# swkrueger/Thrifty

Hardware: AMD Instinct MI355X
Metric: IQ blocks/sec (16384-sample, 1024-chip template) (higher is better)
Workload: dtype f32; 1 GPU; BASELINE configs[1]: block_len=16384 history=4096 1023-chip Gold template, dense, 1048576 blocks/GPU resident in HBM as u8 IQ; variant=default, blocks_per_launch_batch=32768, templates=1, thresholds=15*snr, parallelism=block-shard x1, handles_per_gpu=2, detections_gathered=1048576

## Files before the change

### include/thrifty_hip.h

```cpp
#ifndef THRIFTY_HIP_H
#define THRIFTY_HIP_H

#include <stddef.h>
#include <stdint.h>

#ifdef __cplusplus
extern "C" {
#endif

#define THR_ABI_VERSION 11

#define THR_OK 0
#define THR_ERR_ARG (-1)
#define THR_ERR_DEVICE (-2)
#define THR_ERR_STATE (-3)
#define THR_ERR_INDEX (-4)

#define THR_FLAG_CARRIER 1u
#define THR_FLAG_CORR 2u
#define THR_FLAG_INDEX_ERROR 4u

#define THR_FLAG_FIT_UNCONVERGED 16u
#define THR_FLAG_INT_OFFSET 8u

// ... 168 lines not shown
int thr_run_gate_card(thr_handle* h, const char* text, size_t text_len, const thr_gate_run_opts* opts,
                      thr_gate_run_stats* stats);

typedef struct thr_extract thr_extract;
int thr_extract_create(thr_handle* h, double max_offset, thr_extract** out);
void thr_extract_destroy(thr_extract* x);
int thr_extract_reset(thr_extract* x);
int thr_extract_feed(thr_extract* x, const void* samples, int format, const int64_t* block_idx,
                     const double* timestamps, size_t n_blocks, thr_record* out);
int thr_extract_feed_card(thr_extract* x, const char* text, size_t text_len, const int64_t* payload_off,
                          const int64_t* block_idx, const double* timestamps, size_t n_blocks, thr_record* out);
int thr_extract_feed_stream(thr_extract* x, const uint8_t* stream, size_t n_bytes, int64_t first_block_idx,
                            const double* timestamps, thr_record* out, size_t out_capacity, size_t* n_blocks_out);
int thr_extract_submit_card(thr_extract* x, const char* text, size_t text_len, const int64_t* payload_off,
                            const int64_t* block_idx, const double* timestamps, size_t n_blocks, thr_record* out,
                            uint64_t* ticket);
int thr_extract_submit_stream(thr_extract* x, const uint8_t* stream, size_t n_bytes, int64_t first_block_idx,
                              double timestamp, thr_record* out, size_t out_capacity, size_t* n_blocks_out,
                              uint64_t* ticket);
int thr_extract_result(thr_extract* x, thr_record* best, double* timestamp, double* template_out, size_t capacity,
                       uint64_t* n_qualifying);
int thr_run_extract_card(thr_handle* h, const char* text, size_t text_len, const thr_run_opts* opts,
                         thr_extract* x, thr_run_stats* stats);
int thr_run_extract_stream(thr_handle* h, const uint8_t* stream, size_t n_bytes, int64_t first_block_idx,
                           const thr_run_opts* opts, thr_extract* x, thr_run_stats* stats);

typedef struct thr_survey thr_survey;
int thr_survey_create(thr_handle* h, int integrate, thr_survey** out);
void thr_survey_destroy(thr_survey* s);
int thr_survey_reset(thr_survey* s);
int thr_survey_shift(const thr_survey* s, int* shift);
int thr_survey_pending(const thr_survey* s, uint64_t* blocks_fed, uint64_t* blocks_in_open_interval);
int thr_survey_feed(thr_survey* s, const uint8_t* samples, size_t n_blocks, uint64_t* sums, uint64_t* spec_sum,
                    uint64_t* hist, size_t cap_intervals, size_t* n_intervals);
int thr_survey_feed_stream(thr_survey* s, const uint8_t* stream, size_t n_bytes, uint64_t* sums, size_t sums_capacity,
                           size_t* n_blocks, uint64_t* spec_sum, uint64_t* hist, size_t cap_intervals,
                           size_t* n_intervals);
int thr_debug_survey_geometry(const thr_survey* s, int* tile_blocks, int* workgroups, int* fused);

typedef struct thr_chip_record {
    int32_t sample;
    uint32_t flags;
    float energy, noise;
    double offset;
} thr_chip_record;
int thr_chipscan(thr_handle* h, const void* samples, int format, size_t n_blocks,
                 const uint8_t* chips, int n_chips,
                 const int32_t* lengths, size_t n_lengths,
                 thr_chip_record* out, thr_record* carrier_out );
int thr_debug_chipscan_geometry(thr_handle* h, size_t n_lengths, int* candidates_per_chunk, int* paired);
int thr_debug_chipscan_budget(thr_handle* h, size_t bank_bytes);
int thr_debug_chipscan_times(thr_handle* h, double* ms_out );

int thr_get_settings(const thr_handle* h, thr_settings* out);

int thr_compact_device(thr_handle* h, const thr_record* d_in, size_t n_records,
                       thr_record* d_out, size_t* n_kept);

#define THR_N_KERNEL_SLOTS 5
int thr_profile_enable(thr_handle* h, int on);
int thr_profile_read(thr_handle* h, double ms[THR_N_KERNEL_SLOTS],
                     int64_t launches[THR_N_KERNEL_SLOTS]);
const char* thr_kernel_name(int slot);

int thr_debug_correlate_geom(thr_handle* h, int* rows_lo, int* rows_hi);
#define THR_WHY_SECTIONED 0
#define THR_WHY_PATH 1
#define THR_WHY_VARIANT 2
#define THR_WHY_STDDEV 3
#define THR_WHY_GEOMETRY 4
#define THR_WHY_BLOCK_LEN 5
typedef struct thr_path_info {
    int32_t n_sections, section_len;
    int32_t rows_lo, rows_hi;
    int32_t why_unsectioned;
    int32_t n_templates;
    char carrier_kernel[48];
    char correlate_kernel[48];
    char text[256];
} thr_path_info;
int thr_get_path_info(thr_handle* h, thr_path_info* out);

int thr_debug_sections(thr_handle* h, int* n_sections, int* section_len);
int thr_debug_window(thr_handle* h, size_t out[4]);
int thr_debug_window_times(thr_handle* h, double out[6]);
int thr_debug_pipe_times(thr_handle* h, double out[16]);
int thr_debug_live_resources(int64_t out[4]);
int thr_debug_fft(thr_handle* h, const void* samples, int format, size_t n_blocks,
                  float* spectra_out );
int thr_debug_stage(thr_handle* h, const void* samples, int format, size_t n_blocks,
                    int template_id, float* shifted_fft_out ,
                    float* corr_out );
int thr_debug_stage_offsets(thr_handle* h, const void* samples, int format, size_t n_blocks,
                            int template_id, const double* carrier_offset ,
                            float* shifted_fft_out, float* corr_out);

typedef struct thr_freq_range {
    int32_t rxid;
    int32_t txid;
    double lo;
    double hi;
} thr_freq_range;

int thr_identify(int device_id, size_t n, const int32_t* rxid, const int32_t* block,
                 const double* timestamp, const int32_t* carrier_bin, const double* carrier_offset,
                 const double* energy, const thr_freq_range* map, size_t n_map, int32_t* txid_out,
                 uint8_t* keep_out, int64_t* kept_order_out, size_t* n_kept_out);

int thr_match(int device_id, size_t n, const int32_t* rxid, const int32_t* txid,
              const double* timestamp, const double* energy, double window, int min_match,
              int64_t* match_ptr_out, int64_t* match_idx_out, size_t* n_matches_out,
              int64_t* miss_out, size_t* n_misses_out,
              int64_t* collision_out, size_t* n_collisions_out);
int thr_debug_match_times(double* ms_out );

int thr_tdoa(int device_id, size_t n_det, const int32_t* rx, const double* timestamp, const double* soa,
             const double* energy, const double* noise, size_t n_matches, const int64_t* match_ptr,
             const int64_t* match_idx, const int32_t* match_beacon, int n_rx, int n_beacons,
             const double* dist, double window, double sample_rate, int deg, size_t n_tasks,
             int32_t* row_rx_out, int64_t* row_det_out, double* row_val_out, size_t* n_rows_out,
             int64_t* group_id_out, int64_t* group_ptr_out, size_t* n_groups_out,
             int64_t* fail_out, size_t* n_fail_out, int32_t* n_window_out, int32_t* n_kept_out);
int thr_debug_tdoa_times(double* ms_out );

#define THR_POS_OK 0
#define THR_POS_UNDERDETERMINED 1
#define THR_POS_UNCONVERGED 2
#define THR_POS_AT_BOUND 3
#define THR_POS_NONFINITE 4
int thr_pos(int device_id, size_t n_groups, const int64_t* group_ptr, const int32_t* row_rx0,
            const int32_t* row_rx1, const double* row_tdoa, const double* row_snr, int n_rx, int dims,
            const double* rx_coords, const int32_t* first_two_rx, const double* x0, int max_iter,
            double* pos_out, double* dop_out, double* snr_out, int32_t* status_out, int32_t* iters_out);
int thr_debug_pos_times(double* ms_out );

typedef struct thr_post_settings {
    const thr_freq_range* map;
    size_t n_map;
    double match_window;
    int32_t min_match;
    int32_t n_rx;
    const int32_t* rx_ids;
    int32_t dims;
    int32_t n_beacons;
    const double* rx_coords;
    int32_t first_two_rx[2];
    const int32_t* beacon_ids;
    const double* dist;
    double tdoa_window;
    double sample_rate;
    int32_t deg;
    int32_t max_iter;
    double x0[2];
    int32_t tdoa_as_text;
    int32_t reserved;
} thr_post_settings;
typedef struct thr_post_counts {
    size_t kept, matches, match_entries, misses, collisions, tasks, rows, groups, failures;
} thr_post_counts;
typedef struct thr_post thr_post;
#define THR_POST_TXID 0
#define THR_POST_KEEP 1
#define THR_POST_KEPT_ORDER 2
#define THR_POST_MATCH_PTR 3
#define THR_POST_MATCH_IDX 4
#define THR_POST_MISSES 5
// ... 65 lines not shown
```

### thrifty_amd/_native.py

```python
from __future__ import annotations

import atexit
import ctypes as C
import os
import weakref

import numpy as np

HERE = os.path.dirname(os.path.abspath(__file__))
LIB_PATH = os.environ.get("THRIFTY_HIP_LIB") or os.path.join(HERE, "libthriftyhip.so")

THR_IN_U8 = 0
THR_IN_C64 = 1
FLAG_CARRIER = 1
FLAG_CORR = 2
FLAG_INDEX_ERROR = 4
FLAG_INT_OFFSET = 8
FLAG_FIT_UNCONVERGED = 16
N_KERNEL_SLOTS = 5

ABI_VERSION = 11

EXPORTS = [
    "thr_abi_version", "thr_last_error", "thr_create", "thr_destroy", "thr_detect",
    "thr_create_preshift", "thr_create_fastdet", "thr_create_ex", "thr_plan_sections", "thr_host_register", "thr_host_unregister", "thr_input_window", "thr_detect_card", "thr_detect_stream", "thr_detect_stream_device", "thr_detect_device", "thr_sync", "thr_set_stream", "thr_compact_device",
    "thr_profile_enable", "thr_profile_read", "thr_kernel_name", "thr_debug_fft",
    "thr_debug_stage", "thr_debug_stage_offsets", "thr_identify", "thr_frame_card",
    "thr_submit", "thr_submit_card", "thr_submit_stream", "thr_collect", "thr_inputs_consumed", "thr_poll",
    "thr_set_stream_default", "thr_format_toad",
    "thr_run_card", "thr_run_stream", "thr_get_settings", "thr_input_window_ex", "thr_input_window_release", "thr_detect_offsets", "thr_set_wait_mode", "thr_debug_window", "thr_debug_window_times", "thr_debug_correlate_geom", "thr_debug_sections", "thr_debug_pipe_times", "thr_get_path_info",
    "thr_gate", "thr_gate_stream", "thr_gate_card", "thr_gate_slot_stride", "thr_format_card",
    "thr_run_gate_stream", "thr_run_gate_card",
    "thr_extract_create", "thr_extract_destroy", "thr_extract_reset", "thr_extract_feed", "thr_extract_feed_card",
    "thr_extract_feed_stream", "thr_extract_submit_card", "thr_extract_submit_stream", "thr_extract_result",
    "thr_run_extract_card", "thr_run_extract_stream",
    "thr_match", "thr_debug_match_times",
    "thr_tdoa", "thr_debug_tdoa_times",
    "thr_pos", "thr_debug_pos_times",
    "thr_postdetect", "thr_post_fetch", "thr_post_free", "thr_debug_post_times",
    "thr_debug_live_resources",
    "thr_survey_create", "thr_survey_destroy", "thr_survey_reset", "thr_survey_shift", "thr_survey_pending",
    "thr_survey_feed", "thr_survey_feed_stream", "thr_debug_survey_geometry",
    "thr_chipscan", "thr_debug_chipscan_geometry", "thr_debug_chipscan_budget", "thr_debug_chipscan_times",
    "thr_toadstats", "thr_tstats_fetch", "thr_tstats_free", "thr_debug_toadstats_times", "thr_debug_toadstats_geometry",
]
ERR_ARG, ERR_DEVICE, ERR_STATE, ERR_INDEX = -1, -2, -3, -4
VARIANT_DEFAULT, VARIANT_PRESHIFT, VARIANT_FASTDET, VARIANT_GATE = 0, 1, 2, 3
INTERPOLATORS = {"parabolic": 0, "none": 1, "gaussian": 2, "cosine": 3}
PATHS = {"auto": 0, "multipass": 1, "unsectioned": 2, "generic_rows": 3, "unsectioned_generic_rows": 4}
MAX_IN_FLIGHT = 3
TOAD_LINE_MAX = 384
CARD_HEADER_MAX = 48


class ThrSettings(C.Structure):
    _fields_ = [
        ("block_len", C.c_int32), ("history_len", C.c_int32),
        ("n_templates", C.c_int32), ("template_len", C.c_int32),
        ("templates", C.POINTER(C.c_double)),
        ("carrier_len", C.c_int32), ("carrier_window", C.c_int32 * 2),
        ("carrier_thresh", C.c_double * 3), ("corr_thresh", C.c_double * 3),
        ("device_id", C.c_int32), ("max_batch", C.c_int32),
    ]


class ThrPathInfo(C.Structure):
    _fields_ = [
        ("n_sections", C.c_int32), ("section_len", C.c_int32), ("rows_lo", C.c_int32), ("rows_hi", C.c_int32),
        ("why_unsectioned", C.c_int32), ("n_templates", C.c_int32),
        ("carrier_kernel", C.c_char * 48), ("correlate_kernel", C.c_char * 48), ("text", C.c_char * 256),
    ]


WHY_UNSECTIONED = ("sectioned", "path", "variant", "stddev", "geometry", "block_len")


class ThrRunOpts(C.Structure):
    _fields_ = [
        ("struct_bytes", C.c_uint32), ("batch_blocks", C.c_int32), ("out_fd", C.c_int32),
        ("with_rxid", C.c_int32), ("rxid", C.c_int64), ("with_txid", C.c_int32),
        ("carrier_offset_mode", C.c_int32), ("timestamp", C.c_double),
        ("rec_out", C.c_void_p), ("rec_capacity", C.c_size_t),
    ]


class ThrRunStats(C.Structure):
    _fields_ = [
        ("blocks", C.c_uint64), ("detections", C.c_uint64), ("batches", C.c_uint64),
        ("bytes_in", C.c_uint64), ("text_bytes", C.c_uint64), ("index_error_at", C.c_uint64),
        ("index_error_block", C.c_int64), ("index_error_bin", C.c_int32), ("reserved_", C.c_int32),
        ("total_s", C.c_double), ("frame_s", C.c_double), ("submit_s", C.c_double), ("wait_s", C.c_double),
        ("format_s", C.c_double), ("write_s", C.c_double),
    ]

    def as_dict(self):
        return {name: getattr(self, name) for name, _ in self._fields_ if name != "reserved_"}


class ThrGateRunOpts(C.Structure):
    _fields_ = [
        ("struct_bytes", C.c_uint32), ("batch_blocks", C.c_int32), ("out_fd", C.c_int32), ("skip", C.c_int32),
        ("timestamp", C.c_double), ("rec_out", C.c_void_p), ("rec_capacity", C.c_size_t),
    ]


class ThrGateRunStats(C.Structure):
    _fields_ = [
        ("blocks", C.c_uint64), ("passed", C.c_uint64), ("batches", C.c_uint64), ("bytes_in", C.c_uint64),
        ("text_bytes", C.c_uint64), ("total_s", C.c_double), ("frame_s", C.c_double), ("gate_s", C.c_double),
        ("wait_s", C.c_double), ("format_s", C.c_double), ("write_s", C.c_double),
    ]

    def as_dict(self):
# ... 636 lines not shown
        if buf is None:
            _check(self._lib, self._lib.thr_input_window(self._h, None, 0))
            self._window = None
            return
        if getattr(self, "_window", None) is not None:
            _check(self._lib, self._lib.thr_input_window(self._h, None, 0))
            self._window = None
        arr = np.frombuffer(buf, dtype=np.uint8)
        _check(self._lib, self._lib.thr_input_window_ex(self._h, arr.ctypes.data, arr.size,
                                                        int(populate_threads), int(segment_bytes)))
        self._window = arr

    def input_window_release(self):
        self._lib.thr_input_window_release.argtypes = [C.c_void_p]
        _check(self._lib, self._lib.thr_input_window_release(self._h))

    def _run_opts(self, out_fd, rxid, with_txid, carrier_offset_mode, batch_blocks, rec_out, timestamp=None):
        o = ThrRunOpts()
        o.struct_bytes = C.sizeof(ThrRunOpts)
        o.batch_blocks = int(batch_blocks or 0)
        o.out_fd = -1 if out_fd is None else int(out_fd)
        o.with_rxid, o.rxid = (0, 0) if rxid is None else (1, int(rxid))
        o.with_txid = int(bool(with_txid))
        o.carrier_offset_mode = int(carrier_offset_mode)
        o.timestamp = float("nan") if timestamp is None else float(timestamp)
        if rec_out is not None:
            assert rec_out.dtype == RECORD_DTYPE and rec_out.flags.c_contiguous
            o.rec_out, o.rec_capacity = rec_out.ctypes.data, rec_out.size
        return o

    def _run_done(self, rc, stats):
        out = stats.as_dict()
        out["index_error"] = rc == ERR_INDEX
        if rc != 0 and rc != ERR_INDEX:
            raise NativeError("libthriftyhip: %s (code %d)" % (self._lib.thr_last_error().decode(), rc),
                              rc, out)
        return out

    def _run(self, data, call):
        buf = np.frombuffer(data, dtype=np.uint8)
        st = ThrRunStats()
        rc = call(buf.ctypes.data if buf.size else None, buf.size, C.byref(st))
        del buf
        return self._run_done(rc, st)

    def run_card(self, text, out_fd=None, rxid=None, with_txid=False, carrier_offset_mode=0,
                 batch_blocks=0, rec_out=None):
        o = self._run_opts(out_fd, rxid, with_txid, carrier_offset_mode, batch_blocks, rec_out)
        return self._run(text, lambda ptr, n, st: self._lib.thr_run_card(self._h, ptr, n, C.byref(o), st))

    def run_stream(self, stream, first_block_idx=0, out_fd=None, rxid=None, with_txid=False,
                   carrier_offset_mode=0, batch_blocks=0, rec_out=None, timestamp=None):
        o = self._run_opts(out_fd, rxid, with_txid, carrier_offset_mode, batch_blocks, rec_out, timestamp)
        return self._run(stream, lambda ptr, n, st: self._lib.thr_run_stream(self._h, ptr, n, int(first_block_idx),
                                                                             C.byref(o), st))

    def debug_window(self):
        out = (C.c_size_t * 4)()
        self._lib.thr_debug_window.argtypes = [C.c_void_p, C.c_size_t * 4]
        _check(self._lib, self._lib.thr_debug_window(self._h, out))
        return tuple(int(v) for v in out)

    def correlate_geom(self):
        lo, hi = C.c_int(-1), C.c_int(-1)
        self._lib.thr_debug_correlate_geom.argtypes = [C.c_void_p, C.POINTER(C.c_int), C.POINTER(C.c_int)]
        _check(self._lib, self._lib.thr_debug_correlate_geom(self._h, C.byref(lo), C.byref(hi)))
        return lo.value, hi.value

    def path_info(self):
        info = ThrPathInfo()
        self._lib.thr_get_path_info.argtypes = [C.c_void_p, C.POINTER(ThrPathInfo)]
        _check(self._lib, self._lib.thr_get_path_info(self._h, C.byref(info)))
        return {"n_sections": info.n_sections, "section_len": info.section_len,
                "rows": (info.rows_lo, info.rows_hi), "why_unsectioned": WHY_UNSECTIONED[info.why_unsectioned],
                "n_templates": info.n_templates, "carrier_kernel": info.carrier_kernel.decode(),
                "correlate_kernel": info.correlate_kernel.decode(), "text": info.text.decode()}

    def sections(self):
        n, ln = C.c_int(0), C.c_int(0)
        self._lib.thr_debug_sections.argtypes = [C.c_void_p, C.POINTER(C.c_int), C.POINTER(C.c_int)]
        _check(self._lib, self._lib.thr_debug_sections(self._h, C.byref(n), C.byref(ln)))
        return n.value, ln.value

    def debug_pipe_times(self):
        out = (C.c_double * 16)()
        self._lib.thr_debug_pipe_times.argtypes = [C.c_void_p, C.c_double * 16]
        _check(self._lib, self._lib.thr_debug_pipe_times(self._h, out))
        keys = ("grow_s", "h2d_s", "meta_s", "launch_s", "d2h_s", "chunks", "event_s", "fill_s")
        res = dict(zip(keys, (float(v) for v in out[:8])))
        res.update(("max_" + k, float(v)) for k, v in zip(keys, out[8:]) if k != "chunks")
        return res

    def debug_window_times(self):
        out = (C.c_double * 6)()
        self._lib.thr_debug_window_times.argtypes = [C.c_void_p, C.c_double * 6]
        _check(self._lib, self._lib.thr_debug_window_times(self._h, out))
        keys = ("populate_s", "register_s", "unregister_s", "acquire_wait_s", "acquire_waits", "pageable_copies")
        return dict(zip(keys, (float(v) for v in out)))

    def set_wait_mode(self, sleeping):
        self._lib.thr_set_wait_mode.argtypes = [C.c_void_p, C.c_int]
        _check(self._lib, self._lib.thr_set_wait_mode(self._h, int(bool(sleeping))))

    def collect(self, ticket):
        _check(self._lib, self._lib.thr_collect(self._h, ticket.id))
        ticket.keep = None
        return ticket.out

    def inputs_consumed(self, ticket):
        _check(self._lib, self._lib.thr_inputs_consumed(self._h, ticket.id))
        ticket.keep = None

    def poll(self, ticket):
        done = C.c_int(0)
        _check(self._lib, self._lib.thr_poll(self._h, ticket.id, C.byref(done)))
        return bool(done.value)

    def detect_stream_device(self, d_stream, n_blocks, d_out, d_block_idx=None):
        _check(self._lib, self._lib.thr_detect_stream_device(self._h, d_stream, d_block_idx,
                                                             n_blocks, d_out))

    def detect_device(self, d_samples, fmt, n_blocks, d_out, d_block_idx=None):
        _check(self._lib, self._lib.thr_detect_device(self._h, d_samples, fmt, d_block_idx,
                                                      n_blocks, d_out))

    def compact_device(self, d_in, n_records, d_out):
        kept = C.c_size_t(0)
        _check(self._lib, self._lib.thr_compact_device(self._h, d_in, n_records, d_out,
                                                       C.byref(kept)))
        return kept.value

    def sync(self):
        _check(self._lib, self._lib.thr_sync(self._h))

    def set_stream(self, stream_ptr):
        if not stream_ptr:
            _check(self._lib, self._lib.thr_set_stream_default(self._h))
        else:
            _check(self._lib, self._lib.thr_set_stream(self._h, stream_ptr))

    def use_own_stream(self):
        _check(self._lib, self._lib.thr_set_stream(self._h, None))

    def profile_enable(self, every=1):
        _check(self._lib, self._lib.thr_profile_enable(self._h, int(every)))

    def profile_read(self):
        ms = (C.c_double * N_KERNEL_SLOTS)()
        cnt = (C.c_int64 * N_KERNEL_SLOTS)()
        _check(self._lib, self._lib.thr_profile_read(self._h, ms, cnt))
        return {self._lib.thr_kernel_name(i).decode(): (ms[i], cnt[i])
                for i in range(N_KERNEL_SLOTS)}

    def debug_fft(self, blocks):
        a, fmt = self._as_input(blocks)
        out = np.zeros((a.shape[0], self.block_len), dtype=np.complex64)
        _check(self._lib, self._lib.thr_debug_fft(self._h, a.ctypes.data, fmt, a.shape[0],
                                                  out.ctypes.data))
        return out

    def debug_stage(self, blocks, template_id=0, carrier_offset=None):
        a, fmt = self._as_input(blocks)
        xhat = np.zeros((a.shape[0], self.block_len), dtype=np.complex64)
        corr = np.zeros((a.shape[0], self.block_len), dtype=np.complex64)
        off = None
        if carrier_offset is not None:
# ... 475 lines not shown
```

### thrifty_amd/csrc/detect16k_sec.hip

```cpp
#include <hip/hip_runtime.h>

#include <algorithm>

#include "detect_common.hpp"
#include "fft_regs.hpp"
#include "kernel_util.hpp"
#include "passes_w8.hpp"

namespace thr {

using namespace k16;

namespace {

constexpr int QN = 4096;
constexpr int QR = 4;
constexpr int QA = 8;
constexpr int QT = 128;
constexpr int QDATA = QR * ROW;
constexpr int Q_DYN = 128, Q_PH = 192, Q_NPH = 98;
constexpr size_t QLDS = size_t(QDATA) * sizeof(cpx) + 1024;
#ifndef THR_Q_MULTI_FORM
#define THR_Q_MULTI_FORM 1
#endif
constexpr int Q_MULTI_FORM = THR_Q_MULTI_FORM;

template <int FMT>
struct RawQ;

template <>
struct RawQ<THR_IN_U8> {
    unsigned q[QR * QA / 2];
    __device__ __forceinline__ void load(const void* __restrict__ sec, int t) {
        const unsigned char* p = static_cast<const unsigned char*>(sec) + unsigned(t) * (QA * 2);
#pragma unroll
        for (int n1 = 0; n1 < QR; ++n1)
            __builtin_memcpy(&q[n1 * (QA / 2)], p + n1 * 2048, QA * 2);
    }
    __device__ __forceinline__ void pair(int n1, int i, cpx& a, cpx& b) const {
        const unsigned w = q[n1 * (QA / 2) + i];
        constexpr float sc = 1.0f / 128.0f, of = -127.4f / 128.0f;
        a = __builtin_elementwise_fma(cpx{float(w & 0xffu), float((w >> 8) & 0xffu)}, cpx{sc, sc}, cpx{of, of});
        b = __builtin_elementwise_fma(cpx{float((w >> 16) & 0xffu), float(w >> 24)}, cpx{sc, sc}, cpx{of, of});
    }
};

template <>
struct RawQ<THR_IN_C64> {
    const f4* p;
    __device__ __forceinline__ void load(const void* __restrict__ sec, int t) {
        p = reinterpret_cast<const f4*>(sec) + size_t(t) * (QA / 2);
    }
    __device__ __forceinline__ void pair(int n1, int i, cpx& a, cpx& b) const {
        const f4 w = p[n1 * 512 + i];
        a = cpx{w.x, w.y};
        b = cpx{w.z, w.w};
    }
};

template <class RAW>
__device__ __forceinline__ void q_pass1(cpx* lds, const RAW& raw, int t, const float2* __restrict__ rpow,
                                        const cpx (&qk)[QR], const cpx* u) {
    const int m0 = t * QA;
    cpx* out = lds + (m0 >> 5) * CHUNK + (m0 & 31);
    static_for<QA / 2>([&](auto I) {
        constexpr int i = decltype(I)::value;
        cpx v0[QR], v1[QR];
#pragma unroll
        for (int n1 = 0; n1 < QR; ++n1) {
            raw.pair(n1, i, v0[n1], v1[n1]);
            if (n1 != 0) {
                const cpx r = cpx{rpow[n1].x, rpow[n1].y};
                v0[n1] = cmul_uniform(v0[n1], r);
                v1[n1] = cmul_uniform(v1[n1], r);
            }
        }
        dft_reg<QR, -1>(v0);
        dft_reg<QR, -1>(v1);
        static_for<QR>([&](auto K) {
            constexpr int k1 = decltype(K)::value;
            const f4 uu = *reinterpret_cast<const f4*>(u + k1 * QA + 2 * i);
            cpx w0, w1, y0, y1;
            cmul2(qk[k1], cpx{uu.x, uu.y}, qk[k1], cpx{uu.z, uu.w}, w0, w1);
            cmul2(v0[brev(k1, QR)], w0, v1[brev(k1, QR)], w1, y0, y1);
            *reinterpret_cast<f4*>(out + k1 * ROW + 2 * i) = f4{y0.x, y0.y, y1.x, y1.y};
        });
    });
}

__device__ __forceinline__ void q_pass2(cpx* lds, const cpx (&cw)[R2]) {
    const int t = opaque_tid();
    cpx* base = lds + (t >> 5) * ROW + (t & 31);
    cpx v[R2];
#pragma unroll
    for (int n2 = 0; n2 < R2; ++n2) v[n2] = lds_b64(base + n2 * CHUNK);
    dft_reg<R2, -1>(v);
    static_for<R2 / 2>([&](auto K) {
        constexpr int k2 = 2 * decltype(K)::value;
        cpx y0 = v[brev(k2, R2)], y1 = v[brev(k2 + 1, R2)];
        if constexpr (k2 != 0)
            cmul2(y0, cw[k2], y1, cw[k2 + 1], y0, y1);
        else
            y1 = cmul(y1, cw[1]);
        base[k2 * CHUNK] = y0;
        base[(k2 + 1) * CHUNK] = y1;
    });
}

__device__ __forceinline__ void q_passA(cpx* lds, cpx* z, const cpx (&cw)[R2]) {
    const int t = opaque_tid();
    cpx v[R3];
    static_for<R3>([&](auto K) {
        constexpr int k3 = decltype(K)::value;
        v[k3] = z[brev(k3, R3)];
    });
    dft_reg<R3, +1>(v);
    f4* dst = reinterpret_cast<f4*>(lds + (t >> 5) * ROW + (t & 31) * CHUNK);
    static_for<R3 / 2>([&](auto J) {
        constexpr int j = decltype(J)::value;
        cpx y0 = v[brev(2 * j, R3)], y1 = v[brev(2 * j + 1, R3)];
        if constexpr (j != 0)
            cmulc2(y0, cw[2 * j], y1, cw[2 * j + 1], y0, y1);
        else
            y1 = cmulc(y1, cw[1]);
        dst[j] = f4{y0.x, y0.y, y1.x, y1.y};
    });
}

template <int H>
__device__ __forceinline__ void q_cw_half(const f4* __restrict__ ctp, f4 (&w)[R2 / 4]) {
    const char* p = reinterpret_cast<const char*>(ctp);
    const unsigned off = unsigned(opaque_tid() & 31) * 16u;
    static_for<R2 / 4>([&](auto J) {
        constexpr int j = decltype(J)::value;
        w[j] = *reinterpret_cast<const f4*>(p + (off + unsigned((H * (R2 / 4) + j) * 512)));
    });
}

__device__ __forceinline__ void q_pass2_ld(cpx* lds, const f4* __restrict__ ctp) {
// ... 148 lines not shown
        });
    });
}

struct QPhasor {
    cpx wq;
    float ang;
    cpx seg;
};
__device__ __forceinline__ QPhasor q_phasor_fetch(const ShiftParams* __restrict__ sp, int seg,
                                                  const cpx* __restrict__ twn, int t) {
    QPhasor r;
    const int tt = t < Q_NPH ? t : 0;
    const int u = tt - 66;
    const int m = tt < 64 ? 8 * tt : tt < 66 ? 512 * (tt - 64) : (u & 7);
    const int si = sp->si_mod - (tt < 66 ? 0 : 4 * (u >> 3));
    r.wq = twn[(si * m) & (N - 1)];
    r.ang = 6.283185307179586f * (sp->sf_over_n * float(m));
    r.seg = cpx{sp->segc0[seg].x, sp->segc0[seg].y};
    return r;
}
__device__ __forceinline__ void q_phasor_store(const QPhasor& r, int t, cpx* sc_ph) {
    if (t < Q_NPH) {
        float sn, cs;
        sincos_small(r.ang, &sn, &cs);
        cpx v = cmul(cconj(r.wq), cpx{cs, sn});
        if (t >= 64 && t < 66) v = cmul(v, r.seg);
        sc_ph[t] = v;
    }
}

template <int FMT, bool GENERIC_ROWS, int MULTI>
__global__ __launch_bounds__(QT) __attribute__((amdgpu_waves_per_eu(2))) void k_correlate_4k(
    const void* __restrict__ samples, DevCfg cfg, const cpx* __restrict__ ctab,
    const cpx* __restrict__ twn, const f4* __restrict__ tspec, const ShiftParams* __restrict__ shifts,
    const int* __restrict__ work_list, const int* __restrict__ work_count,
    CorrStats* __restrict__ seg_stats, const f4* __restrict__ ctp, f4* __restrict__ park) {
    extern __shared__ __attribute__((aligned(16))) unsigned char smem_raw[];
    cpx* lds = reinterpret_cast<cpx*>(smem_raw);
    unsigned char* sc_red = reinterpret_cast<unsigned char*>(lds + QDATA);
    cpx* sc_ph = reinterpret_cast<cpx*>(sc_red + Q_PH);
    int* sc_dyn = reinterpret_cast<int*>(sc_red + Q_DYN);

    const size_t blk_bytes = cfg.blk_stride;
    const int n_seg = cfg.n_seg;
    const int n_work = *work_count * n_seg;
    constexpr int kSampleBytes = FMT == THR_IN_U8 ? 2 : 8;
    const cpx* gtw = static_cast<const cpx*>(cfg.gtw);
    int parity = 0;

    cpx cw[R2];
    if constexpr (MULTI != 1) {
        const int c = opaque_tid() & 31;
        cw[0] = cpx{1.f, 0.f};
#pragma unroll
        for (int k = 1; k < R2; ++k) cw[k] = ctab[k * 32 + c];
    }
    f4* const slot = MULTI == 2 ? park + size_t(blockIdx.x) * (QN / 2) + opaque_tid() : nullptr;
    const int n_tpl = MULTI ? cfg.n_templates : 1;

    cpx bk[QR];
    {
        const int m0 = opaque_tid() * QA;
        bk[0] = cpx{1.f, 0.f};
#pragma unroll
        for (int k1 = 1; k1 < QR; ++k1) bk[k1] = gtw[k1 * (16 / QR) * 1024 + m0];
    }

    auto item_entry = [&](int wi) -> int { return n_seg == 4 ? wi >> 2 : wi / n_seg; };
    auto item_at = [&](int wi) -> int {
        const int e = item_entry(wi);
        return (work_list[e] << 3) | (wi - e * n_seg);
    };
    auto item_samples = [&](int item) -> const unsigned char* {
        return static_cast<const unsigned char*>(samples) + size_t(item >> 3) * blk_bytes +
               size_t(cfg.seg_start[item & 7]) * kSampleBytes;
    };

    const int G = int(gridDim.x);
    const int tk = n_work <= 2 * G ? 1 : n_seg;
    auto last_of_ticket = [&](int wi) -> bool {
        return tk == 1 ? true : tk == 4 ? ((wi + 1) & 3) == 0 : (wi + 1) % tk == 0;
    };
    bool static_ticket = true;
    int wi0 = int(blockIdx.x) * tk, wi_nxt;
    if (!last_of_ticket(wi0)) {
        wi_nxt = wi0 + 1;
    } else {
        wi_nxt = (int(blockIdx.x) + G) * tk;
        static_ticket = false;
    }
    RawQ<FMT> cur;
    int it_next = wi0 < n_work ? item_at(wi0) : 0;
    int it_next2 = wi_nxt < n_work ? item_at(wi_nxt) : 0;
    int blk_next2 = it_next2 >> 3, seg_next2 = it_next2 & 7;
    if (wi0 < n_work) {
        cur.load(item_samples(it_next), opaque_tid());
        q_phasor_store(q_phasor_fetch(shifts + (it_next >> 3), it_next & 7, twn, opaque_tid()), opaque_tid(), sc_ph);
    }
    __syncthreads();
    int* dyn_ctr = const_cast<int*>(work_count) + 1;
    f4 tq[R3 / 2];
    auto request_tq = [&](int tpl) {
        const char* ts = reinterpret_cast<const char*>(tspec + size_t(tpl) * (QN / 2));
        const unsigned off = unsigned(opaque_tid()) * 16u;
        static_for<R3 / 2>([&](auto J) {
            constexpr int j = decltype(J)::value;
            tq[j] = *reinterpret_cast<const f4*>(ts + (off + unsigned(j * (QT * 16))));
        });
    };
    if constexpr (MULTI != 0) request_tq(0);
    for (int wi = wi0, iter = 0; wi < n_work; ++iter) {
#ifdef THR_DEV
        const bool tl_on = blockIdx.x == 0 && iter == 40 && cfg.timeline != nullptr;
#endif
        THR_STAMP(0);
        const int item = it_next;
        const int b = item >> 3, seg = item & 7;
        const int t = opaque_tid();
        const ShiftParams* sp = shifts + b;
        const bool need_ticket = last_of_ticket(wi_nxt);
        int wi_dyn = 0;
#ifdef THR_Q_STATIC
        (void)dyn_ctr;
        wi_dyn = (wi_nxt + 1) / tk - 1 - G;
#else
        if (t == 0 && need_ticket && !static_ticket) wi_dyn = atomicAdd(dyn_ctr, 1);
#endif
        RawQ<FMT> nxt = cur;
        const bool more = wi_nxt < n_work;
        if (more) {
            it_next = (blk_next2 << 3) | seg_next2;
            nxt.load(item_samples(it_next), t);
        }
        const QPhasor ph = q_phasor_fetch(shifts + (it_next >> 3), it_next & 7, twn, t);
        THR_STAMP(1);
        {
            cpx qk[QR];
            qk[0] = cmul(sc_ph[64 + (t >> 6)], sc_ph[t & 63]);
#pragma unroll
            for (int k1 = 1; k1 < QR; ++k1) qk[k1] = cmul(qk[0], bk[k1]);
            q_pass1(lds, cur, t, sp->rpow, qk, sc_ph + 66);
        }
        cur = nxt;
        THR_STAMP(2);
        if (t == 0)
            *sc_dyn = !need_ticket ? wi_nxt + 1
                                   : (static_ticket ? int(blockIdx.x) + G : 2 * G + wi_dyn) * tk;
        if (need_ticket) static_ticket = false;
        THR_STAMP(3);
        __syncthreads();
        THR_STAMP(4);
        const int wi_nxt2 = __builtin_amdgcn_readfirstlane(*sc_dyn);
        if (wi_nxt2 < n_work) {
            const int e = item_entry(wi_nxt2);
            blk_next2 = work_list[e];
            seg_next2 = wi_nxt2 - e * n_seg;
        }
        wi = wi_nxt;
        wi_nxt = wi_nxt2;
        if (more) q_phasor_store(ph, t, sc_ph);
        if constexpr (MULTI == 0) request_tq(0);
        if constexpr (MULTI == 1)
            q_pass2_ld(lds, ctp);
        else
            q_pass2(lds, cw);
        __builtin_amdgcn_sched_barrier(0);
        THR_STAMP(5);
        cpx z[R3];
        cpx xh[R3];
        fwd_pass3(lds, xh);
        THR_STAMP(6);
        if constexpr (MULTI == 2) {
            static_for<R3 / 2>([&](auto J) {
                constexpr int j = decltype(J)::value;
                slot[j * QT] = f4{xh[brev(2 * j, R3)].x, xh[brev(2 * j, R3)].y, xh[brev(2 * j + 1, R3)].x,
                                  xh[brev(2 * j + 1, R3)].y};
            });
        }
        static_for<R3 / 2>([&](auto J) {
            constexpr int j = decltype(J)::value;
            const f4 q = tq[j];
            cmul2(xh[brev(2 * j, R3)], cpx{q.x, q.y}, xh[brev(2 * j + 1, R3)], cpx{q.z, q.w},
                  z[brev(2 * j, R3)], z[brev(2 * j + 1, R3)]);
        });
      for (int tpl = 0;;) {
        if constexpr (MULTI == 1)
            q_passA_ld(lds, z, ctp);
        else
            q_passA(lds, z, cw);
        __builtin_amdgcn_sched_barrier(0);
        THR_STAMP(7);
        if constexpr (THR_Q_PAIRED_B)
            q_passB<MULTI == 1>(lds, reinterpret_cast<const f4*>(gtw + 16 * 1024));
        else if constexpr (MULTI == 1)
            q_passB_ld(lds, gtw, (opaque_tid() >> 5) * (16 / QR));
        else
            inv_passB<true>(lds, gtw, (opaque_tid() >> 5) * (16 / QR));
        THR_STAMP(8);
        __syncthreads();
        THR_STAMP(9);
        cpx c[QR * QA];
        q_passC(lds, opaque_tid(), c);
        THR_STAMP(10);

        const int w_lo = cfg.seg_lo[seg], w_hi = cfg.seg_hi[seg];
        const int m0 = t * QA;
        float pw[QR * QA];
        float wmax;
        unsigned lag;
        const bool whole_rows = !GENERIC_ROWS && w_lo <= 1 && w_hi >= 3 * 1024 && w_hi <= 3 * 1024 + 1;
        if (whole_rows) {
            float tmax = -1.0f;
            static_for<3 * QA / 2 + 1>([&](auto Q) {
                constexpr int q = 2 * decltype(Q)::value;
                pw[q] = cnorm(c[q]);
                pw[q + 1] = cnorm(c[q + 1]);
            });
            const float e0 = m0 >= w_lo ? pw[0] : -1.f;
            const float e24 = (m0 == 0 && w_hi > 3 * 1024) ? pw[24] : -1.f;
            tmax = __builtin_fmaxf(e0, e24);
            static_for<3 * QA / 2>([&](auto Q) {
                constexpr int q = 2 * decltype(Q)::value;
                if constexpr (q == 0)
                    tmax = __builtin_fmaxf(tmax, pw[1]);
                else
                    tmax = __builtin_fmaxf(tmax, __builtin_fmaxf(pw[q], pw[q + 1]));
            });
#pragma unroll
            for (int q = 3 * QA + 2; q < QR * QA; ++q) pw[q] = 0.f;
            wmax = wave_max_f32(tmax);
            int first = 63;
            first = e24 == wmax ? 24 : first;
            static_for<3 * QA - 1>([&](auto Q) {
                constexpr int q = 3 * QA - 1 - decltype(Q)::value;
                first = pw[q] == wmax ? q : first;
            });
            first = e0 == wmax ? 0 : first;
            lag = first == 63 ? 0xFFFFFFFFu : unsigned((first >> 3) * 1024 + m0 + (first & 7));
        } else {
            const unsigned win_w = unsigned(w_hi - w_lo);
            float ew[QR * QA];
            float tmax = -1.0f;
            static_for<QR * QA / 2>([&](auto Q) {
                constexpr int q = 2 * decltype(Q)::value;
                constexpr int n1 = q / QA, j = q % QA;
                pw[q] = cnorm(c[q]);
                pw[q + 1] = cnorm(c[q + 1]);
                const int n = n1 * 1024 + m0 + j;
                ew[q] = unsigned(n - w_lo) < win_w ? pw[q] : -1.f;
                ew[q + 1] = unsigned(n + 1 - w_lo) < win_w ? pw[q + 1] : -1.f;
                tmax = __builtin_fmaxf(tmax, __builtin_fmaxf(ew[q], ew[q + 1]));
            });
            wmax = wave_max_f32(tmax);
            int first = 63;
            static_for<QR * QA>([&](auto Q) {
                constexpr int q = QR * QA - 1 - decltype(Q)::value;
                first = ew[q] == wmax ? q : first;
            });
            lag = first == 63 ? 0xFFFFFFFFu : unsigned((first >> 3) * 1024 + m0 + (first & 7));
        }
        const unsigned wlag = wave_min_u32(lag);
        unsigned long long best =
            wmax < 0.f ? 0ull : ((unsigned long long)__float_as_uint(wmax) << 32) | (0xFFFFFFFFu - wlag);
        THR_STAMP(11);
        f4 xs0[R3 / 4], xs1[R3 / 4];
        if constexpr (MULTI != 0) {
            __builtin_amdgcn_sched_barrier(0);
            request_tq(tpl + 1 < n_tpl ? tpl + 1 : 0);
#ifndef THR_Q_XS_LATE
            if constexpr (MULTI == 2)
                static_for<R3 / 4>([&](auto J) { xs0[decltype(J)::value] = slot[decltype(J)::value * QT]; });
#endif
        }
        block_reduce_wave_keys<QT / 64>(best, sc_red, parity);
        THR_STAMP(12);
        parity ^= 1;
        const int pk = int(0xFFFFFFFFu - unsigned(best & 0xFFFFFFFFu));
        CorrStats* cs = seg_stats + (size_t(b) * cfg.n_templates + tpl) * n_seg + seg;
#pragma unroll
        for (int d = 0; d < 3; ++d) {
            const int n = pk - 1 + d;
            if (n < 0 || n >= QN) {
                if (t == 0) cs->m2[d] = 0.f;
                continue;
            }
            const int q = __builtin_amdgcn_readfirstlane((n >> 10) * QA + (n & 7));
            float val = 0.f;
            switch (q) {
#define THR_Q_CASE(Q) case Q: val = pw[Q]; break;
                THR_Q_CASE(0) THR_Q_CASE(1) THR_Q_CASE(2) THR_Q_CASE(3) THR_Q_CASE(4) THR_Q_CASE(5) THR_Q_CASE(6) THR_Q_CASE(7)
                THR_Q_CASE(8) THR_Q_CASE(9) THR_Q_CASE(10) THR_Q_CASE(11) THR_Q_CASE(12) THR_Q_CASE(13) THR_Q_CASE(14) THR_Q_CASE(15)
                THR_Q_CASE(16) THR_Q_CASE(17) THR_Q_CASE(18) THR_Q_CASE(19) THR_Q_CASE(20) THR_Q_CASE(21) THR_Q_CASE(22) THR_Q_CASE(23)
                THR_Q_CASE(24) THR_Q_CASE(25) THR_Q_CASE(26) THR_Q_CASE(27) THR_Q_CASE(28) THR_Q_CASE(29) THR_Q_CASE(30) THR_Q_CASE(31)
#undef THR_Q_CASE
            }
            if (((n & 1023) >> 3) == t) cs->m2[d] = val;
        }
        if (t == 0) {
            cs->pm2 = __uint_as_float(unsigned(best >> 32));
            cs->pk = pk;
            cs->sum_mag = 0.f;
            cs->sum_mag2 = 0.f;
        }
        THR_STAMP(13);
        if (++tpl >= n_tpl) break;
        if constexpr (MULTI == 2) {
#ifdef THR_Q_XS_LATE
            static_for<R3 / 4>([&](auto J) { xs0[decltype(J)::value] = slot[decltype(J)::value * QT]; });
#endif
            static_for<R3 / 4>([&](auto J) { xs1[decltype(J)::value] = slot[(R3 / 4 + decltype(J)::value) * QT]; });
            static_for<R3 / 2>([&](auto J) {
                constexpr int j = decltype(J)::value;
                const f4 q = tq[j];
                const f4 x = j < R3 / 4 ? xs0[j % (R3 / 4)] : xs1[j % (R3 / 4)];
                cmul2(cpx{x.x, x.y}, cpx{q.x, q.y}, cpx{x.z, x.w}, cpx{q.z, q.w},
                      z[brev(2 * j, R3)], z[brev(2 * j + 1, R3)]);
            });
        } else {
            static_for<R3 / 2>([&](auto J) {
                constexpr int j = decltype(J)::value;
                const f4 q = tq[j];
                cmul2(xh[brev(2 * j, R3)], cpx{q.x, q.y}, xh[brev(2 * j + 1, R3)], cpx{q.z, q.w},
                      z[brev(2 * j, R3)], z[brev(2 * j + 1, R3)]);
            });
        }
      }
    }
}

typedef void (*correlate4k_fn)(const void*, DevCfg, const cpx*, const cpx*, const f4*, const ShiftParams*,
                               const int*, const int*, CorrStats*, const f4*, f4*);

template <int FMT>
correlate4k_fn pick_4k(const DevCfg& cfg) {
    if (cfg.n_templates > 1)
        return cfg.no_row_geom ? &k_correlate_4k<FMT, true, Q_MULTI_FORM> : &k_correlate_4k<FMT, false, Q_MULTI_FORM>;
    return cfg.no_row_geom ? &k_correlate_4k<FMT, true, 0> : &k_correlate_4k<FMT, false, 0>;
}

}

size_t lds_bytes_4k() { return QLDS; }
size_t park_bytes_4k(int grid) { return Q_MULTI_FORM == 2 ? size_t(grid) * QN * sizeof(cpx) : 0; }

hipError_t launch_correlate_4k(int fmt, const void* samples, const DevCfg& cfg, const float2* tables,
                               const float2* twn, const float4* tspec4k, const ShiftParams* shifts,
                               const int* work_list, const int* work_count, CorrStats* seg_stats,
                               const float4* ctab_pair, float4* park, int grid, hipStream_t stream) {
    correlate4k_fn fn = fmt == THR_IN_U8 ? pick_4k<THR_IN_U8>(cfg) : pick_4k<THR_IN_C64>(cfg);
#ifdef THR_Q_GRIDCAP
    grid = std::min(grid, THR_Q_GRIDCAP);
#endif
    hipLaunchKernelGGL(fn, dim3(grid), dim3(QT), QLDS, stream, samples, cfg,
                       reinterpret_cast<const cpx*>(tables), reinterpret_cast<const cpx*>(twn),
                       reinterpret_cast<const f4*>(tspec4k), shifts, work_list, work_count, seg_stats,
                       reinterpret_cast<const f4*>(ctab_pair), reinterpret_cast<f4*>(park));
    return hipGetLastError();
}

}
```

### thrifty_amd/csrc/handle.hip

```cpp
#include "host_internal.hpp"

#include "card_gate.hpp"

namespace thr {
namespace host {

thread_local std::string g_last_error;

int fail(int code, const char* fmt, ...) {
    char buf[512];
    va_list ap;
    va_start(ap, fmt);
    vsnprintf(buf, sizeof buf, fmt, ap);
    va_end(ap);
    g_last_error = buf;
    return code;
}

}
}

namespace thr {
int fail_msg(int code, const char* fmt, ...) {
    char buf[512];
// ... 276 lines not shown
}

static int create_impl(const thr_settings* s, int preshift_num, thr_handle** out, int variant = -1,
                       int path = THR_PATH_AUTO, int interp = 0);

int thr_create(const thr_settings* s, thr_handle** out) { return create_impl(s, 0, out); }

static int create_fastdet(const thr_settings* s, thr_handle** out, int path) {
    if (!s || !out) return fail(THR_ERR_ARG, "thr_create_fastdet: null argument");
    if (s->n_templates != 1) return fail(THR_ERR_ARG, "the fastdet variant takes exactly one template");
    if (s->carrier_thresh[2] != 0.0 || s->corr_thresh[2] != 0.0)
        return fail(THR_ERR_ARG, "fastdet thresholds are constant + snr * noise_power (no stddev term)");
    if (s->carrier_window[0] < 0 && s->carrier_window[1] >= 0)
        return fail(THR_ERR_ARG, "Carrier frequency window range not supported.");
    return create_impl(s, 1, out, 2, path);
}

static int create_gate(const thr_settings* s, thr_handle** out, int path) {
    if (!s || !out) return fail(THR_ERR_ARG, "thr_create_ex: null argument");
    if (s->n_templates != 0 || s->templates)
        return fail(THR_ERR_ARG, "the gate variant takes no templates (n_templates = 0, templates = NULL)");
    if (s->carrier_thresh[2] != 0.0)
        return fail(THR_ERR_ARG, "the gate threshold is constant + snr * noise_power (no stddev term)");
    const int n = s->block_len;
    int lo = s->carrier_window[0], hi = s->carrier_window[1];
    if (lo < 0 && hi >= 0)
        return fail(THR_ERR_ARG, "Carrier frequency window range not supported.");
    if (lo < 0) lo += n;
    if (hi < 0) hi += n;
    if (n > 0 && (lo < 0 || hi < 0 || lo >= n || hi >= n))
        return fail(THR_ERR_ARG, "Carrier frequency window out of range.");
    return create_impl(s, 0, out, THR_VARIANT_GATE, path);
}

int thr_create_fastdet(const thr_settings* s, thr_handle** out) try {
    return create_fastdet(s, out, THR_PATH_AUTO);
} catch (...) {
    return thr::on_exception("thr_create_fastdet");
}

static int create_preshift(const thr_settings* s, int num_arg, thr_handle** out, int path) {
    const int num_shifts = num_arg & 0xFFFF, interp = (num_arg >> 16) & 0xFFFF;
    if (num_arg < 0 || interp > THR_INTERP_COSINE)
        return fail(THR_ERR_ARG, "unknown carrier interpolator %d", interp);
    if (num_shifts < 1 || num_shifts > 4096)
        return fail(THR_ERR_ARG, "num_shifts %d out of range [1, 4096]", num_shifts);
    if (s && s->n_templates != 1)
        return fail(THR_ERR_ARG, "the preshift variant takes exactly one template");
    return create_impl(s, num_shifts, out, -1, path, interp);
}

int thr_create_preshift(const thr_settings* s, int num_shifts, thr_handle** out) try {
    return create_preshift(s, num_shifts, out, THR_PATH_AUTO);
} catch (...) {
    return thr::on_exception("thr_create_preshift");
}


int thr_debug_correlate_geom(thr_handle* h, int* rows_lo, int* rows_hi) try {
    if (!h || !rows_lo || !rows_hi) return fail(THR_ERR_ARG, "thr_debug_correlate_geom: null argument");
    *rows_lo = *rows_hi = -1;
    int lo = -1, hi = -1;
    bool got = false;
    if (h->fast && !h->preshift_num)
        got = thr::correlate_geom_16k(h->dev, &lo, &hi);
    else if (h->seg)
        got = thr::correlate_geom_seg(h->dev, &lo, &hi);
    if (got) {
        *rows_lo = lo;
        *rows_hi = hi;
    }
    return THR_OK;
} catch (...) {
    return thr::on_exception("thr_debug_correlate_geom");
}

int thr_debug_sections(thr_handle* h, int* n_sections, int* section_len) try {
    if (!h || !n_sections || !section_len) return fail(THR_ERR_ARG, "thr_debug_sections: null argument");
    *n_sections = (h->seg || h->sec4k) ? h->dev.n_seg : 0;
    *section_len = h->sec4k ? 4096 : h->seg ? 16384 : 0;
    return THR_OK;
} catch (...) {
    return thr::on_exception("thr_debug_sections");
}

int thr_get_path_info(thr_handle* h, thr_path_info* out) try {
    if (!h || !out) return fail(THR_ERR_ARG, "thr_get_path_info: null argument");
    std::memset(out, 0, sizeof(*out));
    out->n_templates = h->cfg.n_templates;
    out->n_sections = (h->seg || h->sec4k) ? h->dev.n_seg : 0;
    out->section_len = h->sec4k ? 4096 : h->seg ? 16384 : 0;
    out->why_unsectioned = h->why_unsectioned;
    out->rows_lo = out->rows_hi = -1;
    const int n = h->cfg.block_len;
    const char* car;
    const char* cor;
    if (h->preshift_num && h->fast) {
        car = cor = "k_preshift";
    } else if (h->fast) {
        car = h->dev.car_prune == 1 ? "k_carrier_pruned" : h->dev.car_prune == 2 ? "k_carrier_pruned (pre-shifted window)"
                                                                                  : "k_carrier";
        cor = h->sec4k ? "k_correlate_4k" : "k_correlate";
        if (!h->sec4k) thr::correlate_geom_16k(h->dev, &out->rows_lo, &out->rows_hi);
    } else if (h->lng && !h->preshift_num) {
        const thr::LongCarrierForm form = thr::long_carrier_form(h->dev, false);
        car = form == thr::kLongCarDit          ? "k_carrier_dit+k_select_dit"
              : form == thr::kLongCarSubPruned ? "k_carrier_sub_pruned+k_select"
                                                : "k_carrier_sub+k_select";
        cor = h->seg ? "k_correlate_seg" : "k_correlate_sub";
        if (h->seg) thr::correlate_geom_seg(h->dev, &out->rows_lo, &out->rows_hi);
    } else if (h->small) {
        car = "k_carrier_small";
        cor = "k_correlate_small";
    } else {
        car = "g_* (multi-pass)";
        cor = "g_* (multi-pass)";
    }
    if (thr_is_gate(h)) {
        cor = "none";
        out->rows_lo = out->rows_hi = -1;
    }
    std::snprintf(out->carrier_kernel, sizeof(out->carrier_kernel), "%s", car);
    std::snprintf(out->correlate_kernel, sizeof(out->correlate_kernel), "%s", cor);
    static const char* const why[] = {
        "",
        "the handle was created with an unsectioned / multi-pass kernel path",
        "preshift / fastdet variant: one fused kernel per block",
        "corr_thresh has a stddev term, whose sums run over every kept lag",
        "the unique window of this history / template length needs more sections than pay",
        "this block length has no sectioned form"};
    if (thr_is_gate(h))
        std::snprintf(out->text, sizeof(out->text),
                      "block_len %d, carrier gate: carrier stage %s, then k_gate_verdict + k_b64_encode; no correlate stage",
                      n, car);
    else if (out->n_sections)
        std::snprintf(out->text, sizeof(out->text),
                      "block_len %d, %d template(s): carrier stage %s, correlate stage %s in %d sections of %d samples",
                      n, h->cfg.n_templates, car, cor, out->n_sections, out->section_len);
    else if (out->rows_lo >= 0)
        std::snprintf(out->text, sizeof(out->text),
                      "block_len %d, %d template(s): carrier stage %s, correlate stage %s (window rows %d, %d), "
                      "unsectioned: %s",
                      n, h->cfg.n_templates, car, cor, out->rows_lo, out->rows_hi, why[h->why_unsectioned]);
    else
        std::snprintf(out->text, sizeof(out->text),
                      "block_len %d, %d template(s): carrier stage %s, correlate stage %s, unsectioned: %s", n,
                      h->cfg.n_templates, car, cor, why[h->why_unsectioned]);
    return THR_OK;
} catch (...) {
    return thr::on_exception("thr_get_path_info");
}


int thr_plan_sections(int block_len, int history_len, int template_len, int* n_sections, int* start,
                      int* win_lo, int* win_hi, int* sum_lo, int* sum_hi) try {
    if (!n_sections || !start || !win_lo || !win_hi || !sum_lo || !sum_hi)
        return fail(THR_ERR_ARG, "thr_plan_sections: null argument");
    if (block_len <= 0 || (block_len & (block_len - 1)) || template_len < 1 || template_len > block_len ||
        history_len < template_len - 1 || history_len >= block_len)
        return fail(THR_ERR_ARG, "thr_plan_sections: bad geometry (%d, %d, %d)", block_len, history_len,
                    template_len);
    thr::DevCfg d{};
    d.block_len = block_len;
    d.corr_len = block_len - template_len + 1;
    const int pad = history_len - template_len + 1;
    d.corr_lo = pad / 2;
// ... 338 lines not shown
```

Measured before the change: 17.98 million blocks/s.

## Skip correlating 4k sections whose energy bound cannot beat the block's best peak

```diff
diff --git a/include/thrifty_hip.h b/include/thrifty_hip.h
--- a/include/thrifty_hip.h
+++ b/include/thrifty_hip.h
@@ -274,6 +274,7 @@
 int thr_get_path_info(thr_handle* h, thr_path_info* out);
 
 int thr_debug_sections(thr_handle* h, int* n_sections, int* section_len);
+int thr_debug_section_counts(thr_handle* h, long long* computed, long long* skipped);
 int thr_debug_window(thr_handle* h, size_t out[4]);
 int thr_debug_window_times(thr_handle* h, double out[6]);
 int thr_debug_pipe_times(thr_handle* h, double out[16]);
diff --git a/thrifty_amd/_native.py b/thrifty_amd/_native.py
--- a/thrifty_amd/_native.py
+++ b/thrifty_amd/_native.py
@@ -28,7 +28,7 @@
     "thr_debug_stage", "thr_debug_stage_offsets", "thr_identify", "thr_frame_card",
     "thr_submit", "thr_submit_card", "thr_submit_stream", "thr_collect", "thr_inputs_consumed", "thr_poll",
     "thr_set_stream_default", "thr_format_toad",
-    "thr_run_card", "thr_run_stream", "thr_get_settings", "thr_input_window_ex", "thr_input_window_release", "thr_detect_offsets", "thr_set_wait_mode", "thr_debug_window", "thr_debug_window_times", "thr_debug_correlate_geom", "thr_debug_sections", "thr_debug_pipe_times", "thr_get_path_info",
+    "thr_run_card", "thr_run_stream", "thr_get_settings", "thr_input_window_ex", "thr_input_window_release", "thr_detect_offsets", "thr_set_wait_mode", "thr_debug_window", "thr_debug_window_times", "thr_debug_correlate_geom", "thr_debug_sections", "thr_debug_section_counts", "thr_debug_pipe_times", "thr_get_path_info",
     "thr_gate", "thr_gate_stream", "thr_gate_card", "thr_gate_slot_stride", "thr_format_card",
     "thr_run_gate_stream", "thr_run_gate_card",
     "thr_extract_create", "thr_extract_destroy", "thr_extract_reset", "thr_extract_feed", "thr_extract_feed_card",
@@ -831,6 +831,12 @@
         _check(self._lib, self._lib.thr_debug_sections(self._h, C.byref(n), C.byref(ln)))
         return n.value, ln.value
 
+    def section_counts(self):
+        done, skipped = C.c_longlong(0), C.c_longlong(0)
+        self._lib.thr_debug_section_counts.argtypes = [C.c_void_p, C.POINTER(C.c_longlong), C.POINTER(C.c_longlong)]
+        _check(self._lib, self._lib.thr_debug_section_counts(self._h, C.byref(done), C.byref(skipped)))
+        return done.value, skipped.value
+
     def debug_pipe_times(self):
         out = (C.c_double * 16)()
         self._lib.thr_debug_pipe_times.argtypes = [C.c_void_p, C.c_double * 16]
diff --git a/thrifty_amd/csrc/detect16k_sec.hip b/thrifty_amd/csrc/detect16k_sec.hip
--- a/thrifty_amd/csrc/detect16k_sec.hip
+++ b/thrifty_amd/csrc/detect16k_sec.hip
@@ -28,6 +28,17 @@
 template <int FMT>
 struct RawQ;
 
+__device__ __forceinline__ unsigned q_wave_sum_u32(unsigned v) {
+    v += dpp_u32<DPP_ROW_SHR1, 0xf>(0u, v);
+    v += dpp_u32<DPP_ROW_SHR2, 0xf>(0u, v);
+    v += dpp_u32<DPP_ROW_SHR4, 0xf>(0u, v);
+    v += dpp_u32<DPP_ROW_SHR8, 0xf>(0u, v);
+    v += dpp_u32<DPP_ROW_BCAST15, 0xa>(0u, v);
+    v += dpp_u32<DPP_ROW_BCAST31, 0xc>(0u, v);
+    return unsigned(__builtin_amdgcn_readlane(int(v), 63));
+}
+
+
 template <>
 struct RawQ<THR_IN_U8> {
     unsigned q[QR * QA / 2];
@@ -43,6 +54,21 @@
         a = __builtin_elementwise_fma(cpx{float(w & 0xffu), float((w >> 8) & 0xffu)}, cpx{sc, sc}, cpx{of, of});
         b = __builtin_elementwise_fma(cpx{float((w >> 16) & 0xffu), float(w >> 24)}, cpx{sc, sc}, cpx{of, of});
     }
+    __device__ __forceinline__ unsigned long long wave_esum() const {
+        unsigned s2 = 0, s1 = 0;
+#pragma unroll
+        for (int i = 0; i < QR * QA / 2; ++i) {
+            s2 = __builtin_amdgcn_udot4(q[i], q[i], s2, false);
+            s1 = __builtin_amdgcn_udot4(q[i], 0x01010101u, s1, false);
+        }
+        return ((unsigned long long)q_wave_sum_u32(s1) << 32) | q_wave_sum_u32(s2);
+    }
+    static __device__ __forceinline__ double energy(unsigned long long a, unsigned long long b) {
+        constexpr double c = double(127.4f);
+        const double s2 = double(unsigned(a)) + double(unsigned(b));
+        const double s1 = double(unsigned(a >> 32)) + double(unsigned(b >> 32));
+        return (s2 - 2.0 * c * s1 + 2.0 * QN * c * c) * (1.0 / 16384.0);
+    }
 };
 
 template <>
@@ -55,6 +81,22 @@
         const f4 w = p[n1 * 512 + i];
         a = cpx{w.x, w.y};
         b = cpx{w.z, w.w};
+    }
+    __device__ __forceinline__ unsigned long long wave_esum() const {
+        float s = 0.f;
+#pragma unroll
+        for (int n1 = 0; n1 < QR; ++n1) {
+            f4 w[QA / 2];
+#pragma unroll
+            for (int i = 0; i < QA / 2; ++i) w[i] = p[n1 * 512 + i];
+#pragma unroll
+            for (int i = 0; i < QA / 2; ++i)
+                s = fmaf(w[i].x, w[i].x, fmaf(w[i].y, w[i].y, fmaf(w[i].z, w[i].z, fmaf(w[i].w, w[i].w, s))));
+        }
+        return __float_as_uint(wave_sum(s));
+    }
+    static __device__ __forceinline__ double energy(unsigned long long a, unsigned long long b) {
+        return double(__uint_as_float(unsigned(a))) + double(__uint_as_float(unsigned(b)));
     }
 };
 
@@ -369,6 +411,13 @@
     auto last_of_ticket = [&](int wi) -> bool {
         return tk == 1 ? true : tk == 4 ? ((wi + 1) & 3) == 0 : (wi + 1) % tk == 0;
     };
+    constexpr bool SKIP = MULTI == 0 && !GENERIC_ROWS;
+    auto first_of_ticket = [&](int wi) -> bool {
+        return tk == 1 ? true : tk == 4 ? (wi & 3) == 0 : wi % tk == 0;
+    };
+    const double skip_scale = (1.0 + 1.0 / 128.0) * double(cfg.tmpl_energy[0]);
+    float blk_best = 0.f;
+    int n_done = 0, n_skipped = 0;
     bool static_ticket = true;
     int wi0 = int(blockIdx.x) * tk, wi_nxt;
     if (!last_of_ticket(wi0)) {
@@ -406,6 +455,18 @@
         const int b = item >> 3, seg = item & 7;
         const int t = opaque_tid();
         const ShiftParams* sp = shifts + b;
+        unsigned long long* const sc_en = reinterpret_cast<unsigned long long*>(sc_red + parity * red_slot_bytes<QT / 64>());
+        bool skip = false;
+        if constexpr (SKIP) {
+            if (first_of_ticket(wi)) {
+                blk_best = 0.f;
+            } else {
+                const unsigned long long* en =
+                    reinterpret_cast<const unsigned long long*>(sc_red + (parity ^ 1) * red_slot_bytes<QT / 64>());
+                const double e = RawQ<FMT>::energy(en[0], en[4]);
+                skip = __builtin_amdgcn_readfirstlane(int(skip_scale * e < double(blk_best))) != 0;
+            }
+        }
         const bool need_ticket = last_of_ticket(wi_nxt);
         int wi_dyn = 0;
 #ifdef THR_Q_STATIC
@@ -422,7 +483,7 @@
         }
         const QPhasor ph = q_phasor_fetch(shifts + (it_next >> 3), it_next & 7, twn, t);
         THR_STAMP(1);
-        {
+        if (!skip) {
             cpx qk[QR];
             qk[0] = cmul(sc_ph[64 + (t >> 6)], sc_ph[t & 63]);
 #pragma unroll
@@ -431,14 +492,21 @@
         }
         cur = nxt;
         THR_STAMP(2);
+        if constexpr (SKIP) {
+            if (skip) {
+                const unsigned long long es = cur.wave_esum();
+                if ((t & 63) == 0) sc_en[(t >> 6) * 4] = es;
+                if (more) q_phasor_store(ph, t, sc_ph);
+            }
+        }
         if (t == 0)
-            *sc_dyn = !need_ticket ? wi_nxt + 1
-                                   : (static_ticket ? int(blockIdx.x) + G : 2 * G + wi_dyn) * tk;
+            sc_dyn[parity] = !need_ticket ? wi_nxt + 1
+                                          : (static_ticket ? int(blockIdx.x) + G : 2 * G + wi_dyn) * tk;
         if (need_ticket) static_ticket = false;
         THR_STAMP(3);
         __syncthreads();
         THR_STAMP(4);
-        const int wi_nxt2 = __builtin_amdgcn_readfirstlane(*sc_dyn);
+        const int wi_nxt2 = __builtin_amdgcn_readfirstlane(sc_dyn[parity]);
         if (wi_nxt2 < n_work) {
             const int e = item_entry(wi_nxt2);
             blk_next2 = work_list[e];
@@ -446,6 +514,23 @@
         }
         wi = wi_nxt;
         wi_nxt = wi_nxt2;
+        if constexpr (SKIP) {
+            if (skip) {
+                if (t == 0) {
+                    CorrStats* cs = seg_stats + size_t(b) * cfg.n_templates * n_seg + seg;
+                    cs->pm2 = 0.f;
+                    cs->m2[0] = 0.f;
+                    cs->m2[1] = 0.f;
+                    cs->m2[2] = 0.f;
+                    cs->sum_mag = 0.f;
+                    cs->sum_mag2 = 0.f;
+                    cs->pk = -1;
+                }
+                ++n_skipped;
+                parity ^= 1;
+                continue;
+            }
+        }
         if (more) q_phasor_store(ph, t, sc_ph);
         if constexpr (MULTI == 0) request_tq(0);
         if constexpr (MULTI == 1)
@@ -487,6 +572,12 @@
         THR_STAMP(8);
         __syncthreads();
         THR_STAMP(9);
+        if constexpr (SKIP) {
+            if (tk != 1) {
+                const unsigned long long es = cur.wave_esum();
+                if ((t & 63) == 0) sc_en[(t >> 6) * 4] = es;
+            }
+        }
         cpx c[QR * QA];
         q_passC(lds, opaque_tid(), c);
         THR_STAMP(10);
@@ -590,6 +681,8 @@
             cs->sum_mag = 0.f;
             cs->sum_mag2 = 0.f;
         }
+        if constexpr (SKIP)
+            blk_best = __builtin_fmaxf(blk_best, __uint_as_float(__builtin_amdgcn_readfirstlane(unsigned(best >> 32))));
         THR_STAMP(13);
         if (++tpl >= n_tpl) break;
         if constexpr (MULTI == 2) {
@@ -613,6 +706,13 @@
             });
         }
       }
+        ++n_done;
+    }
+    if constexpr (MULTI == 0) {
+        if (threadIdx.x == 0 && n_done + n_skipped != 0) {
+            atomicAdd(const_cast<int*>(work_count) + 2, n_done);
+            atomicAdd(const_cast<int*>(work_count) + 3, n_skipped);
+        }
     }
 }
 
diff --git a/thrifty_amd/csrc/handle.hip b/thrifty_amd/csrc/handle.hip
--- a/thrifty_amd/csrc/handle.hip
+++ b/thrifty_amd/csrc/handle.hip
@@ -382,6 +382,21 @@
     return THR_OK;
 } catch (...) {
     return thr::on_exception("thr_debug_sections");
+}
+
+int thr_debug_section_counts(thr_handle* h, long long* computed, long long* skipped) try {
+    if (!h || !computed || !skipped) return fail(THR_ERR_ARG, "thr_debug_section_counts: null argument");
+    HIP_TRY(hipSetDevice(h->device));
+    HIP_TRY(hipStreamSynchronize(h->stream));
+    unsigned n[2] = {0u, 0u};
+    HIP_TRY(hipMemcpyAsync(n, h->d_work_count.p + 2, sizeof n, hipMemcpyDeviceToHost, h->stream));
+    HIP_TRY(hipMemsetAsync(h->d_work_count.p + 2, 0, sizeof n, h->stream));
+    HIP_TRY(hipStreamSynchronize(h->stream));
+    *computed = (long long)n[0];
+    *skipped = (long long)n[1];
+    return THR_OK;
+} catch (...) {
+    return thr::on_exception("thr_debug_section_counts");
 }
 
 int thr_get_path_info(thr_handle* h, thr_path_info* out) try {
```

Result: faster. 22.30 million blocks/s (median of 6 runs) (+24.1%).
